# kongan/PL-SLAM-plucker

Measured on AMD Instinct MI355X. Metric: LM iterations/sec (and ms/iter) on local-BA window; final χ² vs g2o, higher is better.
Workload: dtype f64; 1 GPU; C3: 100 KF (10 fixed) / 20000 points / 4000 Plücker lines, 93975+18441 edges; one independent window per GPU; edges=112416, survey_nominal_edges=120000, trials_per_lba=23, factorisation=two-sided column-lane band LDLT (bw 7), parallelism=1 independent windows (1 per GPU)

## Files before the change

### pl-slam-plucker_amd/csrc/plba_dev.hpp

```cpp
#pragma once

#include <hip/hip_runtime.h>
#include <stdint.h>

#include "../../include/plba.h"
#include "plba_math.hpp"

namespace plba {

constexpr int kBlock = 256;
constexpr int kLmBlock = 64;
constexpr int kChunk = 256;
constexpr int kTraceCap = 64;
constexpr int kTile = 32;
constexpr int kBandMax = 27;
constexpr int kBandNT = 768;
__host__ __device__ constexpr int band_nt(int bw) { return bw <= 24 ? kBandNT : 512; }
__host__ __device__ constexpr int band_ur(int bw) { return band_nt(bw) <= 512 ? 6 : 3; }
constexpr int kMaxSpec = 4;
constexpr int kNB = kMaxSpec + 1;

enum LmKind : int32_t {
    kLmG2o = 0,
    kLmLbaPlucker = 1,
    kLmGba = 2,
    kLmLbaEndpoints = 3
};
__host__ __device__ constexpr bool lm_hand_rolled(int32_t k) { return k != kLmG2o; }
__host__ __device__ constexpr bool lm_endpoint_lines(int32_t k) { return k >= kLmGba; }
__host__ __device__ constexpr bool lm_signed_ldlt(int32_t k) { return k == kLmLbaPlucker; }

struct Ctrl {
    double lambda, ni, currentChi, tempChi, rho, scale, maxdiag;
    double chi2_start, lambda_start;
    double chi2_final[2];
    int32_t qmax, accept, broke;
    int32_t solve_ok[kMaxSpec];
    int32_t last_ok, chi_src;
    int32_t spec_w, spec_sticky;
    int32_t stage, n_stages, iter, need_iter;
    int32_t all_done, switch_pending, robust, level;
    int32_t max_iters[2], iters_done[2];
    int32_t stage_robust[2], stage_level[2], stage_classify[2];
    int32_t max_trials, ntrace, any_active, cur;
    int32_t steps;
    int32_t dev_error;
    int32_t hlm;
    int32_t hlm_lin, hlm_solves, hlm_acc;
    int32_t pad[2];
    double hlm_lambda0, hlm_k, hlm_homog, hlm_minerr, hlm_minchg;
    double hlm_nobs;
    double hlm_nobs2;
    double err_prev, dx2;
};

struct Dev {
    int32_t n_kf, n_pt, n_ln, n_lm, Ep, El, E, nf, n;
    int32_t corrected, n_lin_blocks, n_lm_blocks, n_kf_blocks, nblk, ntiles;
    int32_t solve_lds_n;
    int32_t n_lms_blocks;
    Cam cam;
    double huber_pt, huber_ln, tau;
    double *Tb[kNB], *T_init;
    double *Xb[kNB], *X_init;
    double *xk[kNB];
    double *XL[kNB];
    double *Hl6, *bl6;
    int32_t *ln_gidx;
    double *Lpb[kNB];
    double *xpb[kNB], *xlb[kNB], *chi2b[kNB];
    int32_t nbs, nbx;
    int32_t spec_max, spec_policy;
    int32_t slot;
    double lam;
    double *Tc, *Tt, *Xc, *Xt, *Lpc, *Lpt, *xkc, *xkt, *XLc, *XLt;
    double *xp_prev, *xl_prev;
    int32_t *solve_okp;
    int32_t *cnt_rcs;
    int32_t *kf_hidx;
    int32_t *e_lm, *e_kf, *e_hidx;
// ... 242 lines not shown
```

### pl-slam-plucker_amd/csrc/plba_kernels.hpp

```cpp
#pragma once

#include "plba_dev.hpp"

namespace plba {

__global__ __launch_bounds__(kBlock) void k_linearize(Dev d) {
    ITER_GUARD
    __shared__ double sh[kBlock / 64];
    const int e = blockIdx.x * kBlock + threadIdx.x;
    double rc = 0.0;
    const Ctrl *cc = d.ctrl;
    const bool sw = cc->switch_pending;
    const int nxt = cc->stage + 1;
    const int robust = sw ? cc->stage_robust[nxt] : cc->robust;
    double *chi2e = chi2cur(d);
    __shared__ __attribute__((aligned(16))) double stA[kBlock * 12], stc[kBlock * 2], stB[kBlock * 8];
    if (e < d.E) {
        double *A = stA + threadIdx.x * 12, *c = stc + threadIdx.x * 2, *B = stB + threadIdx.x * 8;
        if (sw) {
            const double stale = chi2e[e];
            for (int b = 0; b < d.nbx; ++b)
                if (d.chi2b[b] != chi2e) d.chi2b[b][e] = stale;
            if (cc->stage_classify[nxt]) {
                bool bad = stale > kChi2Thr;
// ... 283 lines not shown
        st_sc1(d.part_max + d.nf + lb, m);
        __hip_atomic_store(d.part_any + lb, anyb, __ATOMIC_RELAXED, __HIP_MEMORY_SCOPE_AGENT);
    }
    mx_out = m;
    any_out = anyb;
}


template <int NT, bool SC1 = false>
__device__ __forceinline__ double pose_combine(const Dev &d, double *H, double *bp) {
    double m = 0.0;
    for (int i = threadIdx.x; i < d.nf * kPP; i += NT) {
        const int h = i / kPP, k = i % kPP;
        const double *src = d.pose_part + (size_t)h * kPoseParts * kPP + k;
        double v = SC1 ? ld_sc1(src) : src[0];
#pragma unroll
        for (int j = 1; j < kPoseParts; ++j) v += SC1 ? ld_sc1(src + j * kPP) : src[j * kPP];
        if (k < 21) {
            int r = 0, rem = k;
            while (rem >= 6 - r) { rem -= 6 - r; ++r; }
            const int cc = r + rem;
            H[(size_t)h * 36 + r * 6 + cc] = v;
            H[(size_t)h * 36 + cc * 6 + r] = v;
            if (r == cc) m = fmax(m, fabs(v));
        } else if (k < 27) {
            bp[(size_t)h * 6 + (k - 21)] = v;
        } else {
            d.pact_w[h] = v;
        }
    }
    return m;
}

__global__ __launch_bounds__(kInitNT) void k_iter_pack(Dev d) {
    ITER_GUARD
    __shared__ double sh[kInitNT / 64];
    double s = 0.0;
    for (int i = threadIdx.x; i < d.n_lin_blocks; i += kInitNT) s += d.part_chi2[i];
    const double chi = block_sum<kInitNT>(s, sh);
    double m = 0.0;
    for (int i = threadIdx.x; i < d.n_lm_blocks; i += kInitNT) m = fmax(m, d.part_max[d.nf + i]);
    const double mx = block_max<kInitNT>(m, sh);
    int any = 0;
    for (int i = threadIdx.x; i < d.n_lm_blocks; i += kInitNT) any |= d.part_any[i];
    any = __syncthreads_or(any);
    double *o = d.red_iter_loc + (size_t)d.nf * 13;
    if (threadIdx.x == 0) {
        o[0] = chi;
        o[1] = any ? 1.0 : 0.0;
    }
    for (int r = threadIdx.x; r < d.nranks; r += kInitNT) o[2 + r] = r == d.rank ? mx : 0.0;
}

__device__ __forceinline__ void iter_init_ctrl(const Dev &d, double chi, double mx, bool any);
template <int NT>
__device__ __forceinline__ void iter_init_body(const Dev &d, double *sh) {
    double chi, mx;
    bool any;
    if (d.sharded) {
        const double *o = d.red_iter + (size_t)d.nf * 13;
        double m = 0.0;
        for (int i = threadIdx.x; i < d.nf * 6; i += NT) m = fmax(m, fabs(d.Hdg[i]));
        for (int r = threadIdx.x; r < d.nranks; r += NT) m = fmax(m, o[2 + r]);
        mx = block_max<NT>(m, sh);
        chi = o[0];
        any = o[1] != 0.0;
    } else {
        double m = pose_combine<NT>(d, d.Hpp_w, d.bp_w);
        double s = 0.0;
        for (int i = threadIdx.x; i < d.n_lin_blocks; i += NT) s += d.part_chi2[i];
        chi = block_sum<NT>(s, sh);
        for (int i = threadIdx.x; i < d.n_lm_blocks; i += NT) m = fmax(m, d.part_max[d.nf + i]);
        mx = block_max<NT>(m, sh);
        int a = 0;
        for (int i = threadIdx.x; i < d.n_lm_blocks; i += NT) a |= d.part_any[i];
        any = __syncthreads_or(a) != 0;
    }
    if (threadIdx.x == 0) iter_init_ctrl(d, chi, mx, any);
}
__device__ __forceinline__ void iter_init_ctrl(const Dev &d, double chi, double mx, bool any) {
    {
        Ctrl *c = d.ctrl;
        if (c->switch_pending) {
            c->switch_pending = 0;
            c->stage += 1;
            c->iter = 0;
            c->robust = c->stage_robust[c->stage];
            c->level = c->stage_level[c->stage];
            if (!any) {
                c->iters_done[c->stage] = -1;
                c->chi2_final[c->stage] = 0.0;
                c->need_iter = 0;
                if (c->stage + 1 < c->n_stages) c->switch_pending = 1;
                else c->all_done = 1;
                return;
            }
        }
        if (lm_hand_rolled(c->hlm)) {
            const double err = chi / (c->hlm == kLmLbaEndpoints && c->iter > 0 ? c->hlm_nobs2 : c->hlm_nobs);
            c->hlm_lin += 1;
            if (c->iter == 0) {
                c->maxdiag = mx;
                c->lambda = c->hlm_lambda0 * (c->hlm == kLmGba ? (double)(long long)mx : mx);
            } else if (fabs(err - c->err_prev) < c->hlm_minchg || err < c->hlm_minerr) {
                if (c->ntrace < kTraceCap)
                    d.trace[c->ntrace++] = plba_iter_trace{c->stage, c->iter, 0, 3, err, err, c->lambda, c->lambda};
                c->currentChi = err;
                c->chi2_final[c->stage] = err;
                c->need_iter = 0;
                c->all_done = 1;
                return;
            }
            c->currentChi = err;
            c->chi2_start = err;
            c->lambda_start = c->lambda;
            c->accept = 0;
            c->need_iter = 0;
            return;
        }
        if (c->iter == 0) {
            c->currentChi = chi;
            c->maxdiag = mx;
            c->lambda = d.tau * mx;
            c->ni = 2.0;
        }
        c->chi2_start = c->currentChi;
        c->lambda_start = c->lambda;
        c->qmax = 0;
        c->accept = 0;
        c->rho = 0.0;
        c->broke = 0;
        c->need_iter = 0;
    }
}
__global__ __launch_bounds__(kInitNT) void k_iter_init(Dev d) {
    ITER_GUARD
    __shared__ double sh[kInitNT / 64];
    iter_init_body<kInitNT>(d, sh);
}

constexpr int kRedGrp = 256;
__device__ __forceinline__ bool iter_init_fast(const Dev &d) {
    const Ctrl *c = d.ctrl;
    return d.fold_init && !d.sharded && !lm_hand_rolled(c->hlm) && !c->switch_pending && c->iter > 0;
}
__global__ __launch_bounds__(kLmBlock) void k_iter_reduce(Dev d) {
    ITER_GUARD
    __shared__ double sh_init[kLmBlock / 64];
    const int b = blockIdx.x, np = kPoseParts * d.nf;
    const int G = (int)gridDim.x, lane = threadIdx.x;
    double sc = 0.0;
    if (d.fold_init && !iter_init_fast(d)) {
        const int lo = (int)((long long)b * d.n_lin_blocks / G), hi = (int)((long long)(b + 1) * d.n_lin_blocks / G);
        for (int i = lo + lane; i < hi; i += kLmBlock) sc += d.part_chi2[i];
    }
    double wmax = 0.0;
    int wany = 0;
    if (b < np) wmax = pose_partial(d, b / kPoseParts, b % kPoseParts);
    else landmark_reduce(d, b - np, wmax, wany);
    if (!d.fold_init) return;
    if (iter_init_fast(d)) return;
    {
        sc = wave_sum(sc);
        if (lane == 0) {
            st_sc1(d.wg_red + 3 * (size_t)b, sc);
            st_sc1(d.wg_red + 3 * (size_t)b + 1, wmax);
            st_sc1(d.wg_red + 3 * (size_t)b + 2, wany ? 1.0 : 0.0);
        }
    }
    constexpr int U = kRedGrp / kLmBlock;
    const int g = b / kRedGrp, gn = min(kRedGrp, G - kRedGrp * g), ng = (G + kRedGrp - 1) / kRedGrp;
    if (!arrive_last(d.cnt + 2 + d.nblk + d.nf + g, gn)) return;
    {
        double cv[U], mv[U], av[U];
#pragma unroll
        for (int u = 0; u < U; ++u) {
            const int k = lane * U + u;
            const double *w = d.wg_red + 3 * (size_t)(kRedGrp * g + min(k, gn - 1));
            cv[u] = ld_sc1(w);
            mv[u] = ld_sc1(w + 1);
            av[u] = ld_sc1(w + 2);
        }
        double c = 0.0, m = 0.0, a = 0.0;
#pragma unroll
        for (int u = 0; u < U; ++u)
            if (lane * U + u < gn) {
                c += cv[u];
                m = fmax(m, mv[u]);
                a = fmax(a, av[u]);
            }
        c = wave_sum(c);
        m = wave_max(m);
        a = wave_max(a);
        if (lane == 0) {
            st_sc1(d.grp_red + 3 * (size_t)g, c);
            st_sc1(d.grp_red + 3 * (size_t)g + 1, m);
            st_sc1(d.grp_red + 3 * (size_t)g + 2, a);
        }
    }
    if (!arrive_last(d.cnt + 1, ng)) return;
    double c = 0.0, m = 0.0, a = 0.0;
    for (int g0 = 0; g0 < ng; g0 += 64) {
        double cg = 0.0, mg = 0.0, ag = 0.0;
        if (g0 + lane < ng) {
            const double *w = d.grp_red + 3 * (size_t)(g0 + lane);
            cg = ld_sc1(w);
            mg = ld_sc1(w + 1);
            ag = ld_sc1(w + 2);
        }
        c += wave_sum(cg);
        m = fmax(m, wave_max(mg));
        a = fmax(a, wave_max(ag));
    }
    (void)sh_init;
    if (lane == 0) iter_init_ctrl(d, c, m, a != 0.0);
}

}

#include "plba_rcs.hpp"
#include "plba_dense.hpp"
#include "plba_band.hpp"
#include "plba_band_cl.hpp"
#include "plba_bcr.hpp"
#include "plba_pgo.hpp"

namespace plba {

__global__ __launch_bounds__(kBlock) void k_pose_update(Dev d0) {
    TRIAL_SLOT(0)
    if (blockIdx.x == 0) pose_update_wg<kBlock>(d, false);
}

__device__ __forceinline__ void lm_chol(const Dev &d, int l, double lam, bool mul, double (&L)[10], double (&g)[4],
                                        double (&S)[4], bool sgn = false) {
    const int DIM = is_point_lm(d, l) ? 3 : 4;
    double H[10];
#pragma unroll
    for (int k = 0; k < 10; ++k) { H[k] = d.Hll[(size_t)l * 10 + k]; L[k] = 0.0; }
#pragma unroll
    for (int k = 0; k < 4; ++k) { g[k] = 0.0; S[k] = 1.0; }
#pragma unroll
    for (int j = 0; j < 4; ++j) {
        if (j < DIM) {
            double sj = H[pk(j, j)] + (mul ? lam * H[pk(j, j)] : lam);
#pragma unroll
            for (int p = 0; p < j; ++p) sj -= (L[pk(j, p)] * S[p]) * L[pk(j, p)];
            const double sg = (sgn && sj < 0.0) ? -1.0 : 1.0;
            S[j] = sg;
            const double djj = 1.0 / sqrt(sg * sj);
            L[pk(j, j)] = djj;
#pragma unroll
            for (int i = j + 1; i < 4; ++i) {
                if (i < DIM) {
                    double t = H[pk(i, j)];
#pragma unroll
                    for (int p = 0; p < j; ++p) t -= L[pk(i, p)] * (L[pk(j, p)] * S[p]);
                    L[pk(i, j)] = (t * djj) * sg;
                }
            }
        }
    }
#pragma unroll
    for (int i = 0; i < 4; ++i) {
        if (i < DIM) {
            double t = d.bl[(size_t)l * 4 + i];
#pragma unroll
            for (int p = 0; p < i; ++p) t -= L[pk(i, p)] * g[p];
// ... 157 lines not shown

constexpr int kLmLanes = 4;
constexpr int kLmsNT = 256;
constexpr int kLmSlots = 1;
struct LmEdge {
    int e, h, kf;
    bool act;
    double info, obs[4], A[12], B[8];
};
__device__ __forceinline__ void lm_load_edge(const Dev &d, int e, LmEdge &s) {
    s.e = e;
    s.h = d.e_hidx[e];
    s.kf = d.e_kf[e];
    s.act = d.e_active[e] != 0;
    s.info = d.e_info[e];
#pragma unroll
    for (int k = 0; k < 4; ++k) s.obs[k] = d.e_obs[(size_t)e * 4 + k];
#pragma unroll
    for (int k = 0; k < 12; ++k) s.A[k] = d.A[(size_t)e * 12 + k];
#pragma unroll
    for (int k = 0; k < 8; ++k) s.B[k] = d.B[(size_t)e * 8 + k];
}
template <bool GBA = false>
__device__ __forceinline__ void lm_hpl_x(const LmEdge &s, const double (&x)[6], double (&u)[4], double (&u45)[2]) {
    double ax0 = 0, ax1 = 0;
#pragma unroll
    for (int k = 0; k < 6; ++k) {
        ax0 += s.A[k] * x[k];
        ax1 += s.A[6 + k] * x[k];
    }
#pragma unroll
    for (int i = 0; i < 4; ++i) u[i] += s.B[i] * ax0 + s.B[4 + i] * ax1;
    if (GBA) {
        u45[0] += s.B[4] * ax0;
        u45[1] += s.B[5] * ax0;
    }
}
__device__ __forceinline__ double lm_eval(const Dev &d, const LmEdge &s, const double *T, bool pt, const double (&X)[4],
                                          const double (&Lp)[6], bool robust, double delta) {
    double err[2];
    if (pt) {
        double z;
        point_error(T, X, s.obs, d.cam, err, z);
    } else {
        line_error(T, Lp, s.obs, d.cam, err);
    }
    const double c2 = err[0] * (s.info * err[0]) + err[1] * (s.info * err[1]);
    d.chi2_last[s.e] = c2;
    double rho0 = c2, rho1;
    if (robust) huber(c2, delta, rho0, rho1);
    return rho0;
}

constexpr int kSpecOff = 0, kSpecAlways = 1, kSpecAfterReject = 2, kSpecSticky = 3;
template <int NT>
__device__ __forceinline__ void decide_body(const Dev &d, double *sh) {
    const int W = d.ctrl->spec_w;
    double tch[kMaxSpec], scl[kMaxSpec];
#pragma unroll
    for (int s = 0; s < kMaxSpec; ++s) {
        tch[s] = scl[s] = 0.0;
        if (s >= W) continue;
        const double *plm = d.part_lm + (size_t)s * sl_lms(d), *plms = d.part_lms + (size_t)s * sl_lms(d);
        const double *pps = d.part_ps + (size_t)s * d.n_ps;
        double a = 0.0, b = 0.0;
        if (!d.sharded) {
            constexpr int U = 8;
            for (int i0 = threadIdx.x; i0 < d.n_lms_blocks; i0 += NT * U) {
                double va[U], vb[U];
#pragma unroll
                for (int u = 0; u < U; ++u) {
                    const int i = i0 + u * NT;
                    const bool ok = i < d.n_lms_blocks;
                    va[u] = ok ? ld_sc1(plm + i) : 0.0;
                    vb[u] = ok ? ld_sc1(plms + i) : 0.0;
                }
#pragma unroll
                for (int u = 0; u < U; ++u) {
                    a += va[u];
                    b += vb[u];
                }
            }
        }
        for (int i = threadIdx.x; i < d.n_ps; i += NT) b += pps[i];
        tch[s] = block_sum<NT>(a, sh);
        scl[s] = block_sum<NT>(b, sh);
    }
    if (d.sharded) {
        tch[0] = d.red_dec[0];
        scl[0] += d.red_dec[1];
    }
    if (threadIdx.x != 0) return;
    Ctrl *c = d.ctrl;
    c->steps += 1;
    if (lm_hand_rolled(c->hlm)) {
        const double lam0 = c->lambda;
        const bool first = c->iter == 0;
        int result = 0;
        c->hlm_solves += 1;
        const bool ok = d.sharded ? d.red_dec[2] == 0.0
                                  : __hip_atomic_load(&c->solve_ok[0], __ATOMIC_RELAXED, __HIP_MEMORY_SCOPE_AGENT) != 0;
        const double dx2 = ok ? scl[0] : 0.0;
        c->dx2 = dx2;
        bool apply;
        if (first) {
            apply = true;
        } else if (c->currentChi > c->err_prev) {
            c->lambda /= c->hlm_k;
            apply = false;
            result = 1;
        } else {
            c->lambda *= c->hlm_k;
            apply = true;
        }
        if (ok) c->last_ok = (c->last_ok + 1) % d.nbx;
        apply = apply && ok;
        if (apply) {
            c->cur = (c->cur + 1) % d.nbs;
            c->hlm_acc += 1;
        }
        if (c->ntrace < kTraceCap)
            d.trace[c->ntrace++] = plba_iter_trace{c->stage, c->iter, 1, result, c->currentChi, c->currentChi, lam0,
                                                   c->lambda};
        c->iters_done[c->stage] += 1;
        c->iter += 1;
        const bool small = !first && sqrt(dx2) < c->hlm_minchg;
        c->err_prev = c->currentChi;
        if (small || c->iter >= c->max_iters[c->stage]) {
            c->chi2_final[c->stage] = c->currentChi;
            c->all_done = 1;
        } else {
            c->need_iter = 1;
        }
        c->spec_w = 1;
        return;
    }
    const int cur0 = c->cur, lo0 = c->last_ok, ch0 = c->chi_src;
    bool any_ok = false, hold = false, trials_go_on = false, done = false;
    c->need_iter = 0;
#pragma unroll
    for (int s = 0; s < kMaxSpec; ++s) {
        if (done || s >= W) continue;
        const bool ok = c->solve_ok[s] != 0;
        if (!ok && any_ok) {
            hold = true;
            done = true;
            continue;
        }
        c->chi_src = (ch0 + 1 + s) % d.nbx;
        if (ok) {
            c->last_ok = (lo0 + 1 + s) % d.nbx;
            any_ok = true;
        }
        double tempChi = tch[s];
        if (!ok) tempChi = 1.7976931348623157e308;
        const double scale = scl[s] + 1e-3;
        const double rho = (c->currentChi - tempChi) / scale;
        c->tempChi = tempChi;
        c->scale = scale;
        c->rho = rho;
        if (rho > 0 && isfinite(tempChi)) {
            double alpha = 1. - pow((2 * rho - 1), 3);
            alpha = fmin(alpha, 2. / 3.);
            const double sf = fmax(1. / 3., alpha);
            c->lambda *= sf;
            c->ni = 2;
            c->currentChi = tempChi;
            c->accept = 1;
            c->qmax += 1;
            c->cur = (cur0 + 1 + s) % d.nbs;
        } else {
            c->lambda *= c->ni;
            c->ni *= 2;
            c->accept = 0;
            c->spec_sticky = 1;
            if (!isfinite(c->lambda)) c->broke = 1;
            else c->qmax += 1;
        }
        const bool again = !c->broke && rho < 0 && c->qmax < c->max_trials;
        if (again) {
            trials_go_on = true;
            continue;
        }
        trials_go_on = false;
        done = true;
        const int terminate = (c->qmax == c->max_trials || rho == 0 || !isfinite(c->lambda)) ? 1 : 0;
        if (c->ntrace < kTraceCap)
            d.trace[c->ntrace++] = plba_iter_trace{c->stage, c->iter, c->qmax, terminate, c->chi2_start, c->currentChi,
                                                   c->lambda_start, c->lambda};
        c->iters_done[c->stage] += 1;
        c->iter += 1;
        if (terminate || c->iter >= c->max_iters[c->stage]) {
            c->chi2_final[c->stage] = c->currentChi;
            c->spec_sticky = 0;
            if (c->stage + 1 < c->n_stages) c->switch_pending = 1;
            else c->all_done = 1;
        } else {
            c->need_iter = 1;
            c->chi2_start = c->currentChi;
            c->lambda_start = c->lambda;
            c->qmax = 0;
            c->accept = 0;
            c->rho = 0.0;
            c->broke = 0;
        }
    }
    int w = 1;
    if (d.spec_max > 1 && !hold) {
        const int pol = d.spec_policy;
        if (pol == kSpecAlways) w = d.spec_max;
        else if (pol == kSpecAfterReject) w = trials_go_on ? d.spec_max : 1;
        else if (pol == kSpecSticky) w = c->spec_sticky ? d.spec_max : 1;
    }
    c->spec_w = w;
}
__global__ __launch_bounds__(kBlock) void k_decide(Dev d) {
    TRIAL_GUARD
    __shared__ double sh[kBlock / 64];
    decide_body<kBlock>(d, sh);
}

__global__ __launch_bounds__(kLmsNT) void k_lm_solve(Dev d0) {
    TRIAL_GUARD_OF(d0)
    __shared__ double sh[kLmsNT / 64];
    const int nslots = d0.ctrl->spec_w;
    if ((int)blockIdx.y >= nslots) {
        if (d0.fold && arrive_last(d0.cnt, (int32_t)(gridDim.x * gridDim.y))) decide_body<kLmsNT>(d0, sh);
        return;
    }
    const Dev d = slot_view(d0, (int)blockIdx.y);
#ifdef PLBA_LMS_STAMPS
#define LMS_T(v) const unsigned long long v = __builtin_readcyclecounter()
#else
#define LMS_T(v)
#endif
    LMS_T(lt0);
    const int gt = blockIdx.x * kLmsNT + threadIdx.x;
    const int l = gt / kLmLanes, q = gt % kLmLanes;
    const bool live = l < d.n_lm;
    const int lc = live ? l : 0;
    const Ctrl *cg = d.ctrl;
    const bool solve = *d.solve_okp != 0;
    const bool robust = cg->robust != 0;
    const double lam = d.lam;
    const bool hlm = cg->hlm != kLmG2o;
    const bool act = live && d.lm_active[lc] != 0;
    const int off0 = d.lm_off[lc], off1 = d.lm_off[lc + 1];
    double Xc[4], bl[4], H[10];
#pragma unroll
    for (int k = 0; k < 4; ++k) Xc[k] = d.Xc[(size_t)lc * 4 + k];
#pragma unroll
    for (int k = 0; k < 4; ++k) bl[k] = d.bl[(size_t)lc * 4 + k];
#pragma unroll
    for (int k = 0; k < 10; ++k) H[k] = d.Hll[(size_t)lc * 10 + k];
    LmEdge sl[kLmSlots];
    bool sv[kLmSlots];
#pragma unroll
    for (int j = 0; j < kLmSlots; ++j) {
        const int e = off0 + q + kLmLanes * j;
        sv[j] = act && e < off1;
        lm_load_edge(d, sv[j] ? e : 0, sl[j]);
    }
    const double *Tt0 = d.Tt;
    double xs[kLmSlots][6], Ts[kLmSlots][12];
#pragma unroll
    for (int j = 0; j < kLmSlots; ++j) {
        const int h = max(sl[j].h, 0);
#pragma unroll
        for (int k = 0; k < 6; ++k) xs[j][k] = d.xp[6 * h + k];
#pragma unroll
        for (int k = 0; k < 12; ++k) Ts[j][k] = Tt0[(size_t)sl[j].kf * 12 + k];
    }
    double chi = 0.0, sc = 0.0;
    double u[4] = {0, 0, 0, 0}, u45[2] = {0, 0};
    const bool gba_ln = cg->hlm >= kLmGba && live && !is_point_lm(d, l);
    if (act && solve && !(d.diag & 4)) {
        if (gba_ln) {
#pragma unroll
            for (int j = 0; j < kLmSlots; ++j)
                if (sv[j] && sl[j].h >= 0) lm_hpl_x<true>(sl[j], xs[j], u, u45);
// ... 137 lines not shown
            }
            if (q == 0) {
#pragma unroll
                for (int i = 0; i < 4; ++i)
                    if (i < DIM) sc += hlm ? x[i] * x[i] : x[i] * (lam * x[i] + bl[i]);
            }
            double X[4] = {0, 0, 0, 0}, Lp[6] = {0, 0, 0, 0, 0, 0};
            if (pt) {
                X[0] = Xc[0] + x[0]; X[1] = Xc[1] + x[1]; X[2] = Xc[2] + x[2]; X[3] = 0.0;
                if (q == 0) {
#pragma unroll
                    for (int i = 0; i < 4; ++i) Xt[i] = X[i];
                }
            } else if (!(d.diag & 1)) {
                Xt[q] = orth_oplus_quad(Xc, x, q, Lp);
                if (q == 0) {
                    double *Lt = d.Lpt + (size_t)(l - d.n_pt) * 8;
#pragma unroll
                    for (int k = 0; k < 6; ++k) Lt[k] = Lp[k];
                }
            }
            const double delta = pt ? d.huber_pt : d.huber_ln;
            if (!(d.diag & 2) && !hlm)
#pragma unroll
            for (int j = 0; j < kLmSlots; ++j)
                if (sv[j] && sl[j].act) chi += lm_eval(d, sl[j], Ts[j], pt, X, Lp, robust, delta);
            for (int e = off0 + q + kLmLanes * kLmSlots; e < off1 && !hlm; e += kLmLanes) {
                if (!d.e_active[e]) continue;
                LmEdge s;
                lm_load_edge(d, e, s);
                chi += lm_eval(d, s, Tt0 + (size_t)s.kf * 12, pt, X, Lp, robust, delta);
            }
        } else {
            if (q == 0) {
#pragma unroll
                for (int i = 0; i < 4; ++i) Xt[i] = Xc[i];
                if (!is_point_lm(d, l)) {
                    const double *Lc = d.Lpc + (size_t)(l - d.n_pt) * 8;
                    double *Lt = d.Lpt + (size_t)(l - d.n_pt) * 8;
#pragma unroll
                    for (int k = 0; k < 6; ++k) Lt[k] = Lc[k];
                }
            }
        }
    }
    LMS_T(lt2);
    const double s2 = block_sum<kLmsNT>(sc, sh);
    const double s1 = block_sum<kLmsNT>(chi, sh);
    if (threadIdx.x == 0) {
        st_sc1(d.part_lms + blockIdx.x, s2);
        st_sc1(d.part_lm + blockIdx.x, s1);
    }
    LMS_T(lt3);
#ifdef PLBA_LMS_STAMPS
    const bool lms_last = d.fold && arrive_last(d.cnt, (int32_t)(gridDim.x * gridDim.y));
    LMS_T(lt4);
    if (lms_last) decide_body<kLmsNT>(d0, sh);
    LMS_T(lt5);
    if (threadIdx.x == 0 && d.stamps) {
        unsigned long long *st = d.stamps + 15 * 8;
        atomicAdd(st + 0, lt1 - lt0);
        atomicAdd(st + 1, lt2 - lt1);
        atomicAdd(st + 2, lt3 - lt2);
        atomicAdd(st + 3, lt4 - lt3);
        if (lms_last) atomicAdd(st + 4, lt5 - lt4);
        atomicAdd(st + 5, 1ull);
        atomicAdd(st + 6, lt4 - lt0);
        if (lms_last) atomicAdd(st + 7, 1ull);
    }
#else
    if (d.fold && arrive_last(d.cnt, (int32_t)(gridDim.x * gridDim.y))) decide_body<kLmsNT>(d0, sh);
#endif
}
__global__ __launch_bounds__(kBlock) void k_decide_pack(Dev d) {
    TRIAL_GUARD
    __shared__ double sh[kBlock / 64];
    double a = 0.0, b = 0.0;
    for (int i = threadIdx.x; i < d.n_lms_blocks; i += kBlock) a += d.part_lm[i];
    for (int i = threadIdx.x; i < d.n_lms_blocks; i += kBlock) b += d.part_lms[i];
    const double ta = block_sum<kBlock>(a, sh);
    const double tb = block_sum<kBlock>(b, sh);
    if (threadIdx.x == 0) {
        d.red_dec_loc[0] = ta;
        d.red_dec_loc[1] = tb;
        d.red_dec_loc[2] = d.ctrl->solve_ok[0] != 0 ? 0.0 : 1.0;
    }
}

__global__ void k_line_pluker(Dev d) {
    const int l = blockIdx.x * blockDim.x + threadIdx.x;
    if (l >= d.n_ln) return;
    const int cur = d.ctrl->cur;
    double L[6];
    orth_to_pluker(d.Xb[cur] + (size_t)(d.n_pt + l) * 4, L);
    double *o = d.Lpb[cur] + (size_t)l * 8;
#pragma unroll
    for (int k = 0; k < 6; ++k) o[k] = L[k];
}

__global__ __launch_bounds__(kBlock) void k_reset_estimates(Dev d) {
    const size_t t = (size_t)blockIdx.x * kBlock + threadIdx.x, nt = (size_t)gridDim.x * kBlock;
    auto copy = [&](double *dst, const double *src, size_t n) {
        for (size_t i = t; i < n; i += nt) dst[i] = src[i];
    };
    auto zero = [&](double *dst, size_t n) {
        for (size_t i = t; i < (n > 0 ? n : 1); i += nt) dst[i] = 0.0;
    };
    copy(d.Tb[0], d.T_init, (size_t)d.n_kf * 12);
    copy(d.Xb[0], d.X_init, (size_t)d.n_lm * 4);
    for (int b = 0; b < d.nbx; ++b) {
        zero(d.xpb[b], (size_t)d.n);
        zero(d.xlb[b], (size_t)d.n_lm * 4);
        zero(d.chi2b[b], (size_t)d.E);
    }
    const size_t lb = d.E > 0 ? (size_t)d.E : 1, lw = lb / 4;
    uint32_t *lv = reinterpret_cast<uint32_t *>(d.e_level);
    for (size_t i = t; i < lw; i += nt) lv[i] = 0u;
    for (size_t i = lw * 4 + t; i < lb; i += nt) d.e_level[i] = 0;
    if (t == 0) {
        d.ctrl->cur = 0;
        d.ctrl->last_ok = 0;
        d.ctrl->chi_src = 0;
    }
}
// ... 77 lines not shown
```

Before: 5474 LM iterations/s.

## Prefetch LM control state before last-block arrival and batch decide reductions

The LM control struct is now loaded into a register snapshot before the last-arriving-block barrier, and the decide/init logic runs on that snapshot, then writes it back once. The decide reduction is restructured to reduce all speculative slots together, with one wave-level sum per slot and a single __syncthreads, replacing a separate block_sum per slot. The aim is to shorten the serial tail run by the last block by taking scattered global loads off the critical path. The snapshot is loaded speculatively by every block, which adds loads and register pressure, and correctness depends on the ctrl fields not changing between the early load and the arrival.

```diff
diff --git a/pl-slam-plucker_amd/csrc/plba_decide.hpp b/pl-slam-plucker_amd/csrc/plba_decide.hpp
--- /dev/null
+++ b/pl-slam-plucker_amd/csrc/plba_decide.hpp
@@ -0,0 +1,284 @@
+#pragma once
+
+#include <math.h>
+#include <stdint.h>
+
+#include "../../include/plba.h"
+
+#if defined(__HIPCC__)
+#define PLBA_HD __host__ __device__ __forceinline__
+#define PLBA_NOUNROLL _Pragma("nounroll")
+#else
+#define PLBA_HD inline
+#define PLBA_NOUNROLL
+#endif
+
+namespace plba {
+
+constexpr int kTraceCap = 64;
+constexpr int kMaxSpec = 4;
+constexpr int kSpecOff = 0, kSpecAlways = 1, kSpecAfterReject = 2, kSpecSticky = 3;
+
+enum LmKind : int32_t {
+    kLmG2o = 0,
+    kLmLbaPlucker = 1,
+    kLmGba = 2,
+    kLmLbaEndpoints = 3
+};
+
+struct DecideSnap {
+    double lambda, ni, currentChi, tempChi, rho, scale, chi2_start, lambda_start, chi2_final[2];
+    int32_t qmax, accept, broke, last_ok, chi_src, spec_w, spec_sticky;
+    int32_t stage, n_stages, iter, need_iter, all_done, switch_pending;
+    int32_t max_iters[2], iters_done[2], max_trials, ntrace, cur, steps;
+    int32_t hlm, hlm_solves, hlm_acc;
+    double hlm_k, hlm_minchg, err_prev, dx2;
+};
+struct DecideIn {
+    int32_t W;
+    double tch[kMaxSpec], scl[kMaxSpec];
+    bool ok[kMaxSpec];
+    int32_t nbs, nbx, spec_max, spec_policy;
+};
+PLBA_HD int32_t at2(const int32_t (&a)[2], int32_t i) { return i ? a[1] : a[0]; }
+PLBA_HD void inc2(int32_t (&a)[2], int32_t i) {
+    if (i) a[1] += 1;
+    else a[0] += 1;
+}
+PLBA_HD void set2(int32_t (&a)[2], int32_t i, int32_t v) {
+    if (i) a[1] = v;
+    else a[0] = v;
+}
+PLBA_HD void set2(double (&a)[2], int32_t i, double v) {
+    if (i) a[1] = v;
+    else a[0] = v;
+}
+template <class T>
+PLBA_HD T at_slot(const T (&a)[kMaxSpec], int s) {
+    static_assert(kMaxSpec == 4, "at_slot selects among four slots");
+    return s == 0 ? a[0] : s == 1 ? a[1] : s == 2 ? a[2] : a[3];
+}
+
+PLBA_HD bool decide_step(DecideSnap &c, const DecideIn &in, plba_iter_trace &tr) {
+    bool traced = false;
+    c.steps += 1;
+    if (c.hlm != kLmG2o) {
+        const double lam0 = c.lambda;
+        const bool first = c.iter == 0;
+        int result = 0;
+        c.hlm_solves += 1;
+        const bool ok = in.ok[0];
+        const double dx2 = ok ? in.scl[0] : 0.0;
+        c.dx2 = dx2;
+        bool apply;
+        if (first) {
+            apply = true;
+        } else if (c.currentChi > c.err_prev) {
+            c.lambda /= c.hlm_k;
+            apply = false;
+            result = 1;
+        } else {
+            c.lambda *= c.hlm_k;
+            apply = true;
+        }
+        if (ok) c.last_ok = (c.last_ok + 1) % in.nbx;
+        apply = apply && ok;
+        if (apply) {
+            c.cur = (c.cur + 1) % in.nbs;
+            c.hlm_acc += 1;
+        }
+        if (c.ntrace < kTraceCap) {
+            tr = plba_iter_trace{c.stage, c.iter, 1, result, c.currentChi, c.currentChi, lam0, c.lambda};
+            c.ntrace += 1;
+            traced = true;
+        }
+        inc2(c.iters_done, c.stage);
+        c.iter += 1;
+        const bool small = !first && sqrt(dx2) < c.hlm_minchg;
+        c.err_prev = c.currentChi;
+        if (small || c.iter >= at2(c.max_iters, c.stage)) {
+            set2(c.chi2_final, c.stage, c.currentChi);
+            c.all_done = 1;
+        } else {
+            c.need_iter = 1;
+        }
+        c.spec_w = 1;
+        return traced;
+    }
+    const int cur0 = c.cur, lo0 = c.last_ok, ch0 = c.chi_src;
+    bool any_ok = false, hold = false, trials_go_on = false, done = false;
+    c.need_iter = 0;
+    PLBA_NOUNROLL
+    for (int s = 0; s < kMaxSpec; ++s) {
+        if (done || s >= in.W) continue;
+        const bool ok = at_slot(in.ok, s);
+        if (!ok && any_ok) {
+            hold = true;
+            done = true;
+            continue;
+        }
+        c.chi_src = (ch0 + 1 + s) % in.nbx;
+        if (ok) {
+            c.last_ok = (lo0 + 1 + s) % in.nbx;
+            any_ok = true;
+        }
+        double tempChi = at_slot(in.tch, s);
+        if (!ok) tempChi = 1.7976931348623157e308;
+        const double scale = at_slot(in.scl, s) + 1e-3;
+        const double rho = (c.currentChi - tempChi) / scale;
+        c.tempChi = tempChi;
+        c.scale = scale;
+        c.rho = rho;
+        if (rho > 0 && isfinite(tempChi)) {
+            double alpha = 1. - pow((2 * rho - 1), 3);
+            alpha = fmin(alpha, 2. / 3.);
+            const double sf = fmax(1. / 3., alpha);
+            c.lambda *= sf;
+            c.ni = 2;
+            c.currentChi = tempChi;
+            c.accept = 1;
+            c.qmax += 1;
+            c.cur = (cur0 + 1 + s) % in.nbs;
+        } else {
+            c.lambda *= c.ni;
+            c.ni *= 2;
+            c.accept = 0;
+            c.spec_sticky = 1;
+            if (!isfinite(c.lambda)) c.broke = 1;
+            else c.qmax += 1;
+        }
+        const bool again = !c.broke && rho < 0 && c.qmax < c.max_trials;
+        if (again) {
+            trials_go_on = true;
+            continue;
+        }
+        trials_go_on = false;
+        done = true;
+        const int terminate = (c.qmax == c.max_trials || rho == 0 || !isfinite(c.lambda)) ? 1 : 0;
+        if (c.ntrace < kTraceCap) {
+            tr = plba_iter_trace{c.stage, c.iter, c.qmax, terminate, c.chi2_start, c.currentChi, c.lambda_start,
+                                 c.lambda};
+            c.ntrace += 1;
+            traced = true;
+        }
+        inc2(c.iters_done, c.stage);
+        c.iter += 1;
+        if (terminate || c.iter >= at2(c.max_iters, c.stage)) {
+            set2(c.chi2_final, c.stage, c.currentChi);
+            c.spec_sticky = 0;
+            if (c.stage + 1 < c.n_stages) c.switch_pending = 1;
+            else c.all_done = 1;
+        } else {
+            c.need_iter = 1;
+            c.chi2_start = c.currentChi;
+            c.lambda_start = c.lambda;
+            c.qmax = 0;
+            c.accept = 0;
+            c.rho = 0.0;
+            c.broke = 0;
+        }
+    }
+    int w = 1;
+    if (in.spec_max > 1 && !hold) {
+        const int pol = in.spec_policy;
+        if (pol == kSpecAlways) w = in.spec_max;
+        else if (pol == kSpecAfterReject) w = trials_go_on ? in.spec_max : 1;
+        else if (pol == kSpecSticky) w = c.spec_sticky ? in.spec_max : 1;
+    }
+    c.spec_w = w;
+    return traced;
+}
+
+struct InitSnap {
+    double lambda, ni, currentChi, rho, maxdiag, chi2_start, lambda_start, chi2_final[2];
+    int32_t qmax, accept, broke, stage, n_stages, iter, need_iter, all_done, switch_pending, robust, level;
+    int32_t iters_done[2], stage_robust[2], stage_level[2], ntrace;
+    int32_t hlm, hlm_lin;
+    double hlm_lambda0, hlm_minerr, hlm_minchg, hlm_nobs, hlm_nobs2, err_prev;
+};
+PLBA_HD bool iter_init_step(InitSnap &c, double chi, double mx, bool any, double tau, plba_iter_trace &tr) {
+    if (c.switch_pending) {
+        c.switch_pending = 0;
+        c.stage += 1;
+        c.iter = 0;
+        c.robust = at2(c.stage_robust, c.stage);
+        c.level = at2(c.stage_level, c.stage);
+        if (!any) {
+            set2(c.iters_done, c.stage, -1);
+            set2(c.chi2_final, c.stage, 0.0);
+            c.need_iter = 0;
+            if (c.stage + 1 < c.n_stages) c.switch_pending = 1;
+            else c.all_done = 1;
+            return false;
+        }
+    }
+    if (c.hlm != kLmG2o) {
+        const double err = chi / (c.hlm == kLmLbaEndpoints && c.iter > 0 ? c.hlm_nobs2 : c.hlm_nobs);
+        c.hlm_lin += 1;
+        if (c.iter == 0) {
+            c.maxdiag = mx;
+            c.lambda = c.hlm_lambda0 * (c.hlm == kLmGba ? (double)(long long)mx : mx);
+        } else if (fabs(err - c.err_prev) < c.hlm_minchg || err < c.hlm_minerr) {
+            bool traced = false;
+            if (c.ntrace < kTraceCap) {
+                tr = plba_iter_trace{c.stage, c.iter, 0, 3, err, err, c.lambda, c.lambda};
+                c.ntrace += 1;
+                traced = true;
+            }
+            c.currentChi = err;
+            set2(c.chi2_final, c.stage, err);
+            c.need_iter = 0;
+            c.all_done = 1;
+            return traced;
+        }
+        c.currentChi = err;
+        c.chi2_start = err;
+        c.lambda_start = c.lambda;
+        c.accept = 0;
+        c.need_iter = 0;
+        return false;
+    }
+    if (c.iter == 0) {
+        c.currentChi = chi;
+        c.maxdiag = mx;
+        c.lambda = tau * mx;
+        c.ni = 2.0;
+    }
+    c.chi2_start = c.currentChi;
+    c.lambda_start = c.lambda;
+    c.qmax = 0;
+    c.accept = 0;
+    c.rho = 0.0;
+    c.broke = 0;
+    c.need_iter = 0;
+    return false;
+}
+
+#define PLBA_DECIDE_WR(F)                                                                                  \
+    F(lambda) F(ni) F(currentChi) F(tempChi) F(rho) F(scale) F(chi2_start) F(lambda_start) F(chi2_final[0]) \
+    F(chi2_final[1]) F(qmax) F(accept) F(broke) F(last_ok) F(chi_src) F(spec_w) F(spec_sticky) F(iter)      \
+    F(need_iter) F(all_done) F(switch_pending) F(iters_done[0]) F(iters_done[1]) F(ntrace) F(cur) F(steps)  \
+    F(hlm_solves) F(hlm_acc) F(err_prev) F(dx2)
+#define PLBA_DECIDE_RD(F) \
+    F(stage) F(n_stages) F(max_iters[0]) F(max_iters[1]) F(max_trials) F(hlm) F(hlm_k) F(hlm_minchg)
+#define PLBA_INIT_WR(F)                                                                                    \
+    F(lambda) F(ni) F(currentChi) F(rho) F(maxdiag) F(chi2_start) F(lambda_start) F(chi2_final[0])          \
+    F(chi2_final[1]) F(qmax) F(accept) F(broke) F(stage) F(iter) F(need_iter) F(all_done)                   \
+    F(switch_pending) F(robust) F(level) F(iters_done[0]) F(iters_done[1]) F(ntrace) F(hlm_lin)
+#define PLBA_INIT_RD(F)                                                                                    \
+    F(n_stages) F(stage_robust[0]) F(stage_robust[1]) F(stage_level[0]) F(stage_level[1]) F(hlm)            \
+    F(hlm_lambda0) F(hlm_minerr) F(hlm_minchg) F(hlm_nobs) F(hlm_nobs2) F(err_prev)
+#define PLBA_SNAP_LD(f) s.f = c->f;
+#define PLBA_SNAP_ST(f) c->f = s.f;
+template <class C>
+PLBA_HD void snap_load(const C *c, DecideSnap &s) { PLBA_DECIDE_WR(PLBA_SNAP_LD) PLBA_DECIDE_RD(PLBA_SNAP_LD) }
+template <class C>
+PLBA_HD void snap_store(C *c, const DecideSnap &s) { PLBA_DECIDE_WR(PLBA_SNAP_ST) }
+template <class C>
+PLBA_HD void snap_load(const C *c, InitSnap &s) { PLBA_INIT_WR(PLBA_SNAP_LD) PLBA_INIT_RD(PLBA_SNAP_LD) }
+template <class C>
+PLBA_HD void snap_store(C *c, const InitSnap &s) { PLBA_INIT_WR(PLBA_SNAP_ST) }
+#undef PLBA_SNAP_LD
+#undef PLBA_SNAP_ST
+
+}
diff --git a/pl-slam-plucker_amd/csrc/plba_dev.hpp b/pl-slam-plucker_amd/csrc/plba_dev.hpp
--- a/pl-slam-plucker_amd/csrc/plba_dev.hpp
+++ b/pl-slam-plucker_amd/csrc/plba_dev.hpp
@@ -4,6 +4,7 @@
 #include <stdint.h>
 
 #include "../../include/plba.h"
+#include "plba_decide.hpp"
 #include "plba_math.hpp"
 
 namespace plba {
@@ -11,21 +12,13 @@
 constexpr int kBlock = 256;
 constexpr int kLmBlock = 64;
 constexpr int kChunk = 256;
-constexpr int kTraceCap = 64;
 constexpr int kTile = 32;
 constexpr int kBandMax = 27;
 constexpr int kBandNT = 768;
 __host__ __device__ constexpr int band_nt(int bw) { return bw <= 24 ? kBandNT : 512; }
 __host__ __device__ constexpr int band_ur(int bw) { return band_nt(bw) <= 512 ? 6 : 3; }
-constexpr int kMaxSpec = 4;
 constexpr int kNB = kMaxSpec + 1;
 
-enum LmKind : int32_t {
-    kLmG2o = 0,
-    kLmLbaPlucker = 1,
-    kLmGba = 2,
-    kLmLbaEndpoints = 3
-};
 __host__ __device__ constexpr bool lm_hand_rolled(int32_t k) { return k != kLmG2o; }
 __host__ __device__ constexpr bool lm_endpoint_lines(int32_t k) { return k >= kLmGba; }
 __host__ __device__ constexpr bool lm_signed_ldlt(int32_t k) { return k == kLmLbaPlucker; }
diff --git a/pl-slam-plucker_amd/csrc/plba_kernels.hpp b/pl-slam-plucker_amd/csrc/plba_kernels.hpp
--- a/pl-slam-plucker_amd/csrc/plba_kernels.hpp
+++ b/pl-slam-plucker_amd/csrc/plba_kernels.hpp
@@ -359,9 +359,37 @@
     for (int r = threadIdx.x; r < d.nranks; r += kInitNT) o[2 + r] = r == d.rank ? mx : 0.0;
 }
 
-__device__ __forceinline__ void iter_init_ctrl(const Dev &d, double chi, double mx, bool any);
+#ifdef PLBA_LMS_STAMPS
+__device__ __forceinline__ unsigned long long tail_clock() {
+    unsigned long long t;
+    __builtin_amdgcn_sched_barrier(0);
+    asm volatile("s_memtime %0\n\ts_waitcnt lgkmcnt(0)" : "=s"(t)::"memory");
+    __builtin_amdgcn_sched_barrier(0);
+    return t;
+}
+__device__ __forceinline__ void tail_stamps(const Dev &d, int row, unsigned long long t0, unsigned long long t1,
+                                            unsigned long long t2) {
+    asm volatile("s_waitcnt vmcnt(0)" ::: "memory");
+    const unsigned long long t3 = tail_clock();
+    if (!d.stamps) return;
+    unsigned long long *st = d.stamps + row * 8;
+    atomicAdd(st + 0, t1 - t0);
+    atomicAdd(st + 1, t2 - t1);
+    atomicAdd(st + 2, t3 - t2);
+    atomicAdd(st + 3, 1ull);
+}
+#define TAIL_T(v) const unsigned long long v = tail_clock()
+#define TAIL_STAMPS(row, a, b, c) tail_stamps(d, row, a, b, c)
+#else
+#define TAIL_T(v)
+#define TAIL_STAMPS(row, a, b, c)
+#endif
+
+__device__ __forceinline__ void iter_init_ctrl(const Dev &d, const InitSnap &c0, double chi, double mx, bool any);
 template <int NT>
 __device__ __forceinline__ void iter_init_body(const Dev &d, double *sh) {
+    InitSnap c0;
+    if (threadIdx.x == 0) snap_load(d.ctrl, c0);
     double chi, mx;
     bool any;
     if (d.sharded) {
@@ -383,62 +411,13 @@
         for (int i = threadIdx.x; i < d.n_lm_blocks; i += NT) a |= d.part_any[i];
         any = __syncthreads_or(a) != 0;
     }
-    if (threadIdx.x == 0) iter_init_ctrl(d, chi, mx, any);
-}
-__device__ __forceinline__ void iter_init_ctrl(const Dev &d, double chi, double mx, bool any) {
-    {
-        Ctrl *c = d.ctrl;
-        if (c->switch_pending) {
-            c->switch_pending = 0;
-            c->stage += 1;
-            c->iter = 0;
-            c->robust = c->stage_robust[c->stage];
-            c->level = c->stage_level[c->stage];
-            if (!any) {
-                c->iters_done[c->stage] = -1;
-                c->chi2_final[c->stage] = 0.0;
-                c->need_iter = 0;
-                if (c->stage + 1 < c->n_stages) c->switch_pending = 1;
-                else c->all_done = 1;
-                return;
-            }
-        }
-        if (lm_hand_rolled(c->hlm)) {
-            const double err = chi / (c->hlm == kLmLbaEndpoints && c->iter > 0 ? c->hlm_nobs2 : c->hlm_nobs);
-            c->hlm_lin += 1;
-            if (c->iter == 0) {
-                c->maxdiag = mx;
-                c->lambda = c->hlm_lambda0 * (c->hlm == kLmGba ? (double)(long long)mx : mx);
-            } else if (fabs(err - c->err_prev) < c->hlm_minchg || err < c->hlm_minerr) {
-                if (c->ntrace < kTraceCap)
-                    d.trace[c->ntrace++] = plba_iter_trace{c->stage, c->iter, 0, 3, err, err, c->lambda, c->lambda};
-                c->currentChi = err;
-                c->chi2_final[c->stage] = err;
-                c->need_iter = 0;
-                c->all_done = 1;
-                return;
-            }
-            c->currentChi = err;
-            c->chi2_start = err;
-            c->lambda_start = c->lambda;
-            c->accept = 0;
-            c->need_iter = 0;
-            return;
-        }
-        if (c->iter == 0) {
-            c->currentChi = chi;
-            c->maxdiag = mx;
-            c->lambda = d.tau * mx;
-            c->ni = 2.0;
-        }
-        c->chi2_start = c->currentChi;
-        c->lambda_start = c->lambda;
-        c->qmax = 0;
-        c->accept = 0;
-        c->rho = 0.0;
-        c->broke = 0;
-        c->need_iter = 0;
-    }
+    if (threadIdx.x == 0) iter_init_ctrl(d, c0, chi, mx, any);
+}
+__device__ __forceinline__ void iter_init_ctrl(const Dev &d, const InitSnap &c0, double chi, double mx, bool any) {
+    InitSnap c = c0;
+    plba_iter_trace tr;
+    if (iter_init_step(c, chi, mx, any, d.tau, tr)) d.trace[c.ntrace - 1] = tr;
+    snap_store(d.ctrl, c);
 }
 __global__ __launch_bounds__(kInitNT) void k_iter_init(Dev d) {
     ITER_GUARD
@@ -505,7 +484,10 @@
             st_sc1(d.grp_red + 3 * (size_t)g + 2, a);
         }
     }
+    InitSnap c0;
+    if (lane == 0) snap_load(d.ctrl, c0);
     if (!arrive_last(d.cnt + 1, ng)) return;
+    TAIL_T(tt0);
     double c = 0.0, m = 0.0, a = 0.0;
     for (int g0 = 0; g0 < ng; g0 += 64) {
         double cg = 0.0, mg = 0.0, ag = 0.0;
@@ -520,7 +502,12 @@
         a = fmax(a, wave_max(ag));
     }
     (void)sh_init;
-    if (lane == 0) iter_init_ctrl(d, c, m, a != 0.0);
+    TAIL_T(tt1);
+    if (lane == 0) {
+        iter_init_ctrl(d, c0, c, m, a != 0.0);
+        TAIL_T(tt2);
+        TAIL_STAMPS(13, tt0, tt1, tt2);
+    }
 }
 
 }
@@ -784,172 +771,95 @@
     return rho0;
 }
 
-constexpr int kSpecOff = 0, kSpecAlways = 1, kSpecAfterReject = 2, kSpecSticky = 3;
 template <int NT>
-__device__ __forceinline__ void decide_body(const Dev &d, double *sh) {
-    const int W = d.ctrl->spec_w;
-    double tch[kMaxSpec], scl[kMaxSpec];
+__device__ __forceinline__ void decide_body(const Dev &d, const DecideSnap &c0, const int W) {
+    TAIL_T(tt0);
+    constexpr int U = 4, NW = NT / 64;
+    __shared__ double sh_dec[2 * kMaxSpec][NW];
+    int32_t okv[kMaxSpec];
+    double a[kMaxSpec], b[kMaxSpec], p0[kMaxSpec];
 #pragma unroll
     for (int s = 0; s < kMaxSpec; ++s) {
-        tch[s] = scl[s] = 0.0;
+        a[s] = b[s] = p0[s] = 0.0;
+        okv[s] = 1;
         if (s >= W) continue;
-        const double *plm = d.part_lm + (size_t)s * sl_lms(d), *plms = d.part_lms + (size_t)s * sl_lms(d);
-        const double *pps = d.part_ps + (size_t)s * d.n_ps;
-        double a = 0.0, b = 0.0;
-        if (!d.sharded) {
-            constexpr int U = 8;
-            for (int i0 = threadIdx.x; i0 < d.n_lms_blocks; i0 += NT * U) {
-                double va[U], vb[U];
+        if (threadIdx.x == 0)
+            okv[s] = __hip_atomic_load(&d.ctrl->solve_ok[s], __ATOMIC_RELAXED, __HIP_MEMORY_SCOPE_AGENT);
+        if ((int)threadIdx.x < d.n_ps) p0[s] = d.part_ps[(size_t)s * d.n_ps + threadIdx.x];
+    }
+    if (!d.sharded) {
+        for (int i0 = threadIdx.x; i0 < d.n_lms_blocks; i0 += NT * U) {
+            double va[kMaxSpec][U], vb[kMaxSpec][U];
+#pragma unroll
+            for (int s = 0; s < kMaxSpec; ++s)
 #pragma unroll
                 for (int u = 0; u < U; ++u) {
                     const int i = i0 + u * NT;
-                    const bool ok = i < d.n_lms_blocks;
-                    va[u] = ok ? ld_sc1(plm + i) : 0.0;
-                    vb[u] = ok ? ld_sc1(plms + i) : 0.0;
-                }
+                    const bool ok = s < W && i < d.n_lms_blocks;
+                    va[s][u] = ok ? ld_sc1(d.part_lm + (size_t)s * sl_lms(d) + i) : 0.0;
+                    vb[s][u] = ok ? ld_sc1(d.part_lms + (size_t)s * sl_lms(d) + i) : 0.0;
+                }
+#pragma unroll
+            for (int s = 0; s < kMaxSpec; ++s)
 #pragma unroll
                 for (int u = 0; u < U; ++u) {
-                    a += va[u];
-                    b += vb[u];
-                }
-            }
-        }
-        for (int i = threadIdx.x; i < d.n_ps; i += NT) b += pps[i];
-        tch[s] = block_sum<NT>(a, sh);
-        scl[s] = block_sum<NT>(b, sh);
+                    a[s] += va[s][u];
+                    b[s] += vb[s][u];
+                }
+        }
+    }
+#pragma unroll
+    for (int s = 0; s < kMaxSpec; ++s) {
+        if (s >= W) continue;
+        b[s] += p0[s];
+        for (int i = threadIdx.x + NT; i < d.n_ps; i += NT) b[s] += d.part_ps[(size_t)s * d.n_ps + i];
+        const double wa = wave_sum(a[s]), wb = wave_sum(b[s]);
+        if ((threadIdx.x & 63) == 0) {
+            sh_dec[2 * s][threadIdx.x >> 6] = wa;
+            sh_dec[2 * s + 1][threadIdx.x >> 6] = wb;
+        }
+    }
+    __syncthreads();
+    if (threadIdx.x != 0) return;
+    DecideIn in;
+    in.W = W;
+#pragma unroll
+    for (int s = 0; s < kMaxSpec; ++s) {
+        in.tch[s] = in.scl[s] = 0.0;
+        in.ok[s] = okv[s] != 0;
+        if (s >= W) continue;
+        double ra = sh_dec[2 * s][0], rb = sh_dec[2 * s + 1][0];
+#pragma unroll
+        for (int w = 1; w < NW; ++w) {
+            ra += sh_dec[2 * s][w];
+            rb += sh_dec[2 * s + 1][w];
+        }
+        in.tch[s] = ra;
+        in.scl[s] = rb;
     }
     if (d.sharded) {
-        tch[0] = d.red_dec[0];
-        scl[0] += d.red_dec[1];
-    }
-    if (threadIdx.x != 0) return;
-    Ctrl *c = d.ctrl;
-    c->steps += 1;
-    if (lm_hand_rolled(c->hlm)) {
-        const double lam0 = c->lambda;
-        const bool first = c->iter == 0;
-        int result = 0;
-        c->hlm_solves += 1;
-        const bool ok = d.sharded ? d.red_dec[2] == 0.0
-                                  : __hip_atomic_load(&c->solve_ok[0], __ATOMIC_RELAXED, __HIP_MEMORY_SCOPE_AGENT) != 0;
-        const double dx2 = ok ? scl[0] : 0.0;
-        c->dx2 = dx2;
-        bool apply;
-        if (first) {
-            apply = true;
-        } else if (c->currentChi > c->err_prev) {
-            c->lambda /= c->hlm_k;
-            apply = false;
-            result = 1;
-        } else {
-            c->lambda *= c->hlm_k;
-            apply = true;
-        }
-        if (ok) c->last_ok = (c->last_ok + 1) % d.nbx;
-        apply = apply && ok;
-        if (apply) {
-            c->cur = (c->cur + 1) % d.nbs;
-            c->hlm_acc += 1;
-        }
-        if (c->ntrace < kTraceCap)
-            d.trace[c->ntrace++] = plba_iter_trace{c->stage, c->iter, 1, result, c->currentChi, c->currentChi, lam0,
-                                                   c->lambda};
-        c->iters_done[c->stage] += 1;
-        c->iter += 1;
-        const bool small = !first && sqrt(dx2) < c->hlm_minchg;
-        c->err_prev = c->currentChi;
-        if (small || c->iter >= c->max_iters[c->stage]) {
-            c->chi2_final[c->stage] = c->currentChi;
-            c->all_done = 1;
-        } else {
-            c->need_iter = 1;
-        }
-        c->spec_w = 1;
-        return;
-    }
-    const int cur0 = c->cur, lo0 = c->last_ok, ch0 = c->chi_src;
-    bool any_ok = false, hold = false, trials_go_on = false, done = false;
-    c->need_iter = 0;
-#pragma unroll
-    for (int s = 0; s < kMaxSpec; ++s) {
-        if (done || s >= W) continue;
-        const bool ok = c->solve_ok[s] != 0;
-        if (!ok && any_ok) {
-            hold = true;
-            done = true;
-            continue;
-        }
-        c->chi_src = (ch0 + 1 + s) % d.nbx;
-        if (ok) {
-            c->last_ok = (lo0 + 1 + s) % d.nbx;
-            any_ok = true;
-        }
-        double tempChi = tch[s];
-        if (!ok) tempChi = 1.7976931348623157e308;
-        const double scale = scl[s] + 1e-3;
-        const double rho = (c->currentChi - tempChi) / scale;
-        c->tempChi = tempChi;
-        c->scale = scale;
-        c->rho = rho;
-        if (rho > 0 && isfinite(tempChi)) {
-            double alpha = 1. - pow((2 * rho - 1), 3);
-            alpha = fmin(alpha, 2. / 3.);
-            const double sf = fmax(1. / 3., alpha);
-            c->lambda *= sf;
-            c->ni = 2;
-            c->currentChi = tempChi;
-            c->accept = 1;
-            c->qmax += 1;
-            c->cur = (cur0 + 1 + s) % d.nbs;
-        } else {
-            c->lambda *= c->ni;
-            c->ni *= 2;
-            c->accept = 0;
-            c->spec_sticky = 1;
-            if (!isfinite(c->lambda)) c->broke = 1;
-            else c->qmax += 1;
-        }
-        const bool again = !c->broke && rho < 0 && c->qmax < c->max_trials;
-        if (again) {
-            trials_go_on = true;
-            continue;
-        }
-        trials_go_on = false;
-        done = true;
-        const int terminate = (c->qmax == c->max_trials || rho == 0 || !isfinite(c->lambda)) ? 1 : 0;
-        if (c->ntrace < kTraceCap)
-            d.trace[c->ntrace++] = plba_iter_trace{c->stage, c->iter, c->qmax, terminate, c->chi2_start, c->currentChi,
-                                                   c->lambda_start, c->lambda};
-        c->iters_done[c->stage] += 1;
-        c->iter += 1;
-        if (terminate || c->iter >= c->max_iters[c->stage]) {
-            c->chi2_final[c->stage] = c->currentChi;
-            c->spec_sticky = 0;
-            if (c->stage + 1 < c->n_stages) c->switch_pending = 1;
-            else c->all_done = 1;
-        } else {
-            c->need_iter = 1;
-            c->chi2_start = c->currentChi;
-            c->lambda_start = c->lambda;
-            c->qmax = 0;
-            c->accept = 0;
-            c->rho = 0.0;
-            c->broke = 0;
-        }
-    }
-    int w = 1;
-    if (d.spec_max > 1 && !hold) {
-        const int pol = d.spec_policy;
-        if (pol == kSpecAlways) w = d.spec_max;
-        else if (pol == kSpecAfterReject) w = trials_go_on ? d.spec_max : 1;
-        else if (pol == kSpecSticky) w = c->spec_sticky ? d.spec_max : 1;
-    }
-    c->spec_w = w;
+        in.tch[0] = d.red_dec[0];
+        in.scl[0] += d.red_dec[1];
+        if (lm_hand_rolled(c0.hlm)) in.ok[0] = d.red_dec[2] == 0.0;
+    }
+    in.nbs = d.nbs;
+    in.nbx = d.nbx;
+    in.spec_max = d.spec_max;
+    in.spec_policy = d.spec_policy;
+    TAIL_T(tt1);
+    DecideSnap c = c0;
+    plba_iter_trace tr;
+    if (decide_step(c, in, tr)) d.trace[c.ntrace - 1] = tr;
+    snap_store(d.ctrl, c);
+    TAIL_T(tt2);
+    TAIL_STAMPS(14, tt0, tt1, tt2);
 }
 __global__ __launch_bounds__(kBlock) void k_decide(Dev d) {
     TRIAL_GUARD
-    __shared__ double sh[kBlock / 64];
-    decide_body<kBlock>(d, sh);
+    const int W = d.ctrl->spec_w;
+    DecideSnap c0;
+    if (threadIdx.x == 0) snap_load(d.ctrl, c0);
+    decide_body<kBlock>(d, c0, W);
 }
 
 __global__ __launch_bounds__(kLmsNT) void k_lm_solve(Dev d0) {
@@ -957,7 +867,11 @@
     __shared__ double sh[kLmsNT / 64];
     const int nslots = d0.ctrl->spec_w;
     if ((int)blockIdx.y >= nslots) {
-        if (d0.fold && arrive_last(d0.cnt, (int32_t)(gridDim.x * gridDim.y))) decide_body<kLmsNT>(d0, sh);
+        if (d0.fold) {
+            DecideSnap c0;
+            if (threadIdx.x == 0) snap_load(d0.ctrl, c0);
+            if (arrive_last(d0.cnt, (int32_t)(gridDim.x * gridDim.y))) decide_body<kLmsNT>(d0, c0, nslots);
+        }
         return;
     }
     const Dev d = slot_view(d0, (int)blockIdx.y);
@@ -1201,10 +1115,12 @@
         st_sc1(d.part_lm + blockIdx.x, s1);
     }
     LMS_T(lt3);
+    DecideSnap c0;
+    if (d.fold && threadIdx.x == 0) snap_load(d0.ctrl, c0);
 #ifdef PLBA_LMS_STAMPS
     const bool lms_last = d.fold && arrive_last(d.cnt, (int32_t)(gridDim.x * gridDim.y));
     LMS_T(lt4);
-    if (lms_last) decide_body<kLmsNT>(d0, sh);
+    if (lms_last) decide_body<kLmsNT>(d0, c0, nslots);
     LMS_T(lt5);
     if (threadIdx.x == 0 && d.stamps) {
         unsigned long long *st = d.stamps + 15 * 8;
@@ -1218,7 +1134,7 @@
         if (lms_last) atomicAdd(st + 7, 1ull);
     }
 #else
-    if (d.fold && arrive_last(d.cnt, (int32_t)(gridDim.x * gridDim.y))) decide_body<kLmsNT>(d0, sh);
+    if (d.fold && arrive_last(d.cnt, (int32_t)(gridDim.x * gridDim.y))) decide_body<kLmsNT>(d0, c0, nslots);
 #endif
 }
 __global__ __launch_bounds__(kBlock) void k_decide_pack(Dev d) {
```

After: 5513 LM iterations/s, median of 6. Within noise of the previous version (+0.7%).
